# YannDubs/lossyless

Measured on AMD Instinct MI355X. Metric: encode_img_per_sec, higher is better.
Workload: dtype f16; 1 GPU; clip_compressor_b005 encode, synthetic 224x224x3 fp16 NHWC, batch=1024/GPU (configs[1]); batch_per_gpu=1024, layout=nhwc, vit_weights=synthetic-seed1, parallelism=image-parallel x1, entropy_group=16, tower_batch=8704, tower_streams=1, distinct_batches=9

## Files before the change

include/lossyless_amd.h:

```cpp
#ifndef LOSSYLESS_AMD_H
#define LOSSYLESS_AMD_H

#include <stddef.h>
#include <stdint.h>

#ifdef __cplusplus
extern "C" {
#endif

#define LLA_OK 0
#define LLA_EINVAL (-1)
#define LLA_ECAP (-2)
#define LLA_EHIP (-3)
#define LLA_EDATA (-4)

#define LLA_ABI_VERSION 4

int lla_abi_version(void);
const char *lla_source_sha(void);
int lla_last_hip_error(void);


int lla_pmf_to_quantized_cdf(const float *pmf, int n, int precision, uint32_t *cdf_out);

// ... 208 lines not shown
int lla_gemm_f32(const float *A, int lda, const float *W, int ldw, const float *bias, float *C, int ldc,
                 int M, int N, int K, int relu, void *stream);

size_t lla_svm_pass_workspace_bytes(int C, int K);
int lla_svm_pass(const void *z, int z_dtype, int ld_z, const int32_t *y, int B, int C, const float *W, const float *b,
                 const float *V, const float *vb, int K, int ld_w, float *out_W, float *out_b, double *out_loss,
                 int accumulate, void *workspace, void *stream);

size_t lla_svm_grid_pass_workspace_bytes(int C, int J);
int lla_svm_grid_pass(const void *z, int z_dtype, int ld_z, const int32_t *y, const int32_t *fold, int B, int C,
                      const float *W, const float *b, const float *V, const float *vb, int J, int ld_w,
                      const int32_t *col_class, const int32_t *col_held, const float *col_cpos, const float *col_cneg,
                      float *out_W, float *out_b, double *out_loss, int accumulate, void *workspace, void *stream);

size_t lla_softmax_pass_workspace_bytes(int C, int K, int B);
int lla_softmax_pass(const void *z, int z_dtype, int ld_z, const int32_t *y, int B, int C, const float *W, const float *b,
                     const float *V, const float *vb, int K, int ld_w, const float *class_weight, float *out_W,
                     float *out_b, double *out_loss, int accumulate, void *workspace, void *stream);

size_t lla_softmax_grid_pass_workspace_bytes(int C, int K, int G);
int lla_softmax_grid_pass(const void *z, int z_dtype, int ld_z, const int32_t *y, const int32_t *fold, int B, int C,
                          const float *W, const float *b, const float *V, const float *vb, int K, int G, int ld_w,
                          const int32_t *group_held, const float *group_class_weight, float *out_W, float *out_b,
                          double *out_loss, int accumulate, void *workspace, void *stream);


int lla_gemm_f32_nn(const float *dY, int ldy, const float *W, int ldw, const float *H, int ldh, float *dX, int ldx,
                    int M, int N, int K, void *stream);
int lla_gemm_f32_tn(const float *dY, int ldy, const float *X, int ldx, float *dW, int ldw, float *db, int M, int N, int K,
                    void *stream);
size_t lla_softmax_xent_workspace_bytes(int B);
int lla_softmax_xent(const float *logits, int ld, const int32_t *y, int B, int K, int Kpad, float scale, float *dlogits,
                     int ldd, double *out_loss, int32_t *out_correct, void *workspace, void *stream);
int lla_adamw_step(float *p, const float *g, float *m, float *v, long long n, double lr, double beta1, double beta2,
                   double eps, double weight_decay, double bias_correction1, double bias_correction2, void *stream);

int lla_conv3x3_relu_f16(const void *in, int n, int H, int W, int pitch, int cin, const void *weights,
                         const float *bias, void *out, int ldc, int cout, void *stream);
int lla_conv3x3_direct_relu_f16(const void *in, int n, int H, int W, int pitch, int cin, const void *weights, int kpad,
                                const void *bias, void *out, int ldc, int cout, int pool, void *stream);
int lla_rn50_bottleneck_f16(const void *x, int n, int H, int W, int pitch, int cin, const void *w1, int k1pad, const void *b1,
                            const void *w2, int k2pad, const void *b2, const void *w3, int k3pad, const void *b3, void *out,
                            int ldo, void *stream);
int lla_conv3x3_rgb_s2_relu_f16(const void *in, int n, int H, int W, const void *weights, int kpad, const void *bias,
                                void *out, int ldc, void *stream);
int lla_patch_embed_f16(const void *images, int layout, int B, const void *conv_w, const float *pos,
                        float *x, void *stream);
int lla_layernorm768(const float *x, size_t row_stride, const float *w, const float *b,
                     void *y16, int rows, void *stream);
size_t lla_gemm_resid_layernorm768_workspace_bytes(int M);
int lla_gemm_resid_layernorm768(const void *A, int lda, const void *W, const float *bias, float *x, const float *gamma,
                                const float *beta, void *h16, int M, int K, int wait_cycles, int rev, void *workspace,
                                void *stream);
int lla_attention50(const void *qkv, void *o, int B, void *stream);

size_t lla_rn50_weights_bytes(void);
int lla_rn50_conv_count(void);
int lla_rn50_conv_desc(int i, int64_t *out8);
int lla_rn50_fused_desc(int stage, int64_t *out8);
int lla_rn50_attnpool_offsets(int64_t *out7);
size_t lla_rn50_workspace_bytes(int chunk);
int lla_rn50_forward(const void *images_nhwc_f16, int B, const void *weights, void *workspace,
                     size_t workspace_bytes, int chunk, void *z_out, void *stream, void *tower);

#ifdef __cplusplus
}
#endif
#endif
```

lossyless_amd/_lib.py:

```python
import ctypes
import os

import torch

_HERE = os.path.dirname(os.path.abspath(__file__))
LIB_PATH = os.environ.get("LLA_LIB") or os.path.join(_HERE, "liblossyless_amd.so")

LLA_OK = 0
LLA_EINVAL, LLA_ECAP, LLA_EHIP, LLA_EDATA = -1, -2, -3, -4
ABI_VERSION = 4
LLA_Z_F16, LLA_Z_F32 = 1, 2
LLA_LAYOUT_NHWC, LLA_LAYOUT_NCHW = 0, 1
LLA_EPI_F16, LLA_EPI_QUICKGELU_F16, LLA_EPI_RESID_F32, LLA_EPI_RELU_F16, LLA_EPI_ADD_RELU_F16 = 0, 1, 2, 4, 5
_ERR = {-1: "LLA_EINVAL", -2: "LLA_ECAP", -3: "LLA_EHIP", -4: "LLA_EDATA"}

VIT_GLOBAL = dict(CONV1_NHWC=0, CONV1_NCHW=1, CLASS_EMB=2, POS_EMB=3, LN_PRE_W=4, LN_PRE_B=5,
                  LN_POST_W=6, LN_POST_B=7, PROJ_T=8)
VIT_LAYER = dict(LN1_W=16, LN1_B=17, QKV_W=18, QKV_B=19, OUT_W=20, OUT_B=21, LN2_W=22, LN2_B=23,
                 FC_W=24, FC_B=25, CPROJ_W=26, CPROJ_B=27)

_vp, _i, _sz = ctypes.c_void_p, ctypes.c_int, ctypes.c_size_t
_SIGNATURES = {
    "lla_abi_version": (_i, []),
    "lla_last_hip_error": (_i, []),
# ... 37 lines not shown
    "lla_preprocess_workspace_bytes": (_sz, [_i, _i]),
    "lla_preprocess_clip": (_i, [_vp, _i, _i, _i, _i, _i, _vp, _vp, _i, _vp, _vp, _i, _vp, _vp, _vp, _sz,
                                 _vp, _vp]),
    "lla_vit_b32_weights_bytes": (_sz, []),
    "lla_vit_b32_param_offset": (_sz, [_i, _i]),
    "lla_vit_b32_param_bytes": (_sz, [_i]),
    "lla_vit_b32_workspace_bytes": (_sz, [_i]),
    "lla_vit_b32_forward": (_i, [_vp, _i, _i, _vp, _vp, _sz, _i, _vp, _vp]),
    "lla_profiler_create": (_i, [ctypes.POINTER(ctypes.c_void_p), _i]),
    "lla_profiler_destroy": (_i, [_vp]),
    "lla_profiler_collect": (_i, [_vp, _vp, _vp, _vp]),
    "lla_vit_b32_forward_profiled": (_i, [_vp, _i, _i, _vp, _vp, _sz, _i, _vp, _vp, _vp]),
    "lla_tower_create": (_i, [ctypes.POINTER(ctypes.c_void_p)]),
    "lla_tower_destroy": (_i, [_vp]),
    "lla_tower_join": (_i, [_vp, _vp]),
    "lla_tower_set_option": (_i, [_vp, _i, _i]),
    "lla_vit_b32_forward_lanes": (_i, [_vp, _vp, _i, _i, _vp, _vp, _sz, _i, _vp, _vp, _i]),
    "lla_vit_b32_forward_gather": (_i, [_vp, _vp, _i, _i, _i, _i, _vp, _vp, _sz, _vp, _vp]),
    "lla_gemm_f16": (_i, [_vp, _vp, _vp, _vp, _i, _i, _i, _i, _vp]),
    "lla_patch_embed_f16": (_i, [_vp, _i, _i, _vp, _vp, _vp, _vp]),
    "lla_gemm_plan": (_i, [_i, _i, _i, _i, _i, _i, _i, _i, _i, _vp, _vp, _vp]),
    "lla_gemm_f16_ex": (_i, [_vp, _i, _vp, _vp, _vp, _i, _vp, _i, _i, _i, _i, _i, _vp]),
    "lla_gemm_f32": (_i, [_vp, _i, _vp, _i, _vp, _vp, _i, _i, _i, _i, _i, _vp]),
    "lla_svm_pass_workspace_bytes": (_sz, [_i, _i]),
    "lla_svm_pass": (_i, [_vp, _i, _i, _vp, _i, _i, _vp, _vp, _vp, _vp, _i, _i, _vp, _vp, _vp, _i, _vp, _vp]),
    "lla_svm_grid_pass_workspace_bytes": (_sz, [_i, _i]),
    "lla_svm_grid_pass": (_i, [_vp, _i, _i, _vp, _vp, _i, _i, _vp, _vp, _vp, _vp, _i, _i, _vp, _vp, _vp, _vp, _vp, _vp, _vp,
                               _i, _vp, _vp]),
    "lla_softmax_pass_workspace_bytes": (_sz, [_i, _i, _i]),
    "lla_softmax_pass": (_i, [_vp, _i, _i, _vp, _i, _i, _vp, _vp, _vp, _vp, _i, _i, _vp, _vp, _vp, _vp, _i, _vp, _vp]),
    "lla_softmax_grid_pass_workspace_bytes": (_sz, [_i, _i, _i]),
    "lla_softmax_grid_pass": (_i, [_vp, _i, _i, _vp, _vp, _i, _i, _vp, _vp, _vp, _vp, _i, _i, _i, _vp, _vp, _vp, _vp, _vp,
                                   _i, _vp, _vp]),
    "lla_gemm_f32_nn": (_i, [_vp, _i, _vp, _i, _vp, _i, _vp, _i, _i, _i, _i, _vp]),
    "lla_gemm_f32_tn": (_i, [_vp, _i, _vp, _i, _vp, _i, _vp, _i, _i, _i, _vp]),
    "lla_softmax_xent_workspace_bytes": (_sz, [_i]),
    "lla_softmax_xent": (_i, [_vp, _i, _vp, _i, _i, _i, ctypes.c_float, _vp, _i, _vp, _vp, _vp, _vp]),
    "lla_adamw_step": (_i, [_vp, _vp, _vp, _vp, ctypes.c_longlong] + [ctypes.c_double] * 7 + [_vp]),
    "lla_conv3x3_relu_f16": (_i, [_vp, _i, _i, _i, _i, _i, _vp, _vp, _vp, _i, _i, _vp]),
    "lla_conv3x3_direct_relu_f16": (_i, [_vp, _i, _i, _i, _i, _i, _vp, _i, _vp, _vp, _i, _i, _i, _vp]),
    "lla_conv3x3_rgb_s2_relu_f16": (_i, [_vp, _i, _i, _i, _vp, _i, _vp, _vp, _i, _vp]),
    "lla_rn50_bottleneck_f16": (_i, [_vp, _i, _i, _i, _i, _i, _vp, _i, _vp, _vp, _i, _vp, _vp, _i, _vp, _vp, _i, _vp]),
    "lla_rn50_weights_bytes": (_sz, []),
    "lla_rn50_conv_count": (_i, []),
    "lla_rn50_conv_desc": (_i, [_i, _vp]),
    "lla_rn50_fused_desc": (_i, [_i, _vp]),
    "lla_rn50_attnpool_offsets": (_i, [_vp]),
    "lla_rn50_workspace_bytes": (_sz, [_i]),
    "lla_rn50_forward": (_i, [_vp, _i, _vp, _vp, _sz, _i, _vp, _vp, _vp]),
    "lla_layernorm768": (_i, [_vp, _sz, _vp, _vp, _vp, _i, _vp]),
    "lla_gemm_resid_layernorm768_workspace_bytes": (_sz, [_i]),
    "lla_gemm_resid_layernorm768": (_i, [_vp, _i, _vp, _vp, _vp, _vp, _vp, _vp, _i, _i, _i, _i, _vp, _vp]),
    "lla_attention50": (_i, [_vp, _vp, _i, _vp]),
}
EXPORTS = tuple(sorted(_SIGNATURES))

_lib = None
_CSRC = os.path.join(_HERE, "csrc")


def tree_sha():
    script = os.path.join(_CSRC, "source_sha.py")
    if not os.path.exists(script):
        return None
    import importlib.util
    spec = importlib.util.spec_from_file_location("_lla_source_sha", script)
    mod = importlib.util.module_from_spec(spec)
    spec.loader.exec_module(mod)
    return mod.source_sha(_CSRC)


def built_sha(path=None):
    import re
    path = path or LIB_PATH
    if not os.path.exists(path):
        return None
    with open(path, "rb") as f:
        m = re.search(rb"LLA_SOURCE_SHA=([0-9a-f]{16})", f.read())
    return m.group(1).decode() if m else None


def stale(path=None):
    path = path or LIB_PATH
    if not os.path.exists(path):
        return f"{path} is missing"
    want, have = tree_sha(), built_sha(path)
    if want is not None and have != want:
        return f"{path} was built from sources {have}, the tree is {want}"
    return None


def ensure_built(path=None):
    import subprocess
    path = path or LIB_PATH
    why = stale(path)
    if why is None:
        return False
    name = os.path.basename(path)
    if os.path.dirname(os.path.abspath(path)) == os.path.join(_HERE, "variants"):
        raise RuntimeError(f"{why}: rebuild it with the DEFS it was made with (make -C lossyless_amd/csrc variant NAME=... DEFS=...)")
    target = {"liblossyless_amd.so": [], "liblossyless_amd_ablation.so": ["ablation"], "liblossyless_amd_probes.so": ["probes"]}.get(name)
    if target is None or _lib is not None:
        raise RuntimeError(why)
    subprocess.check_call(["make", "-j8", "-C", _CSRC, *target])
    return True

# ... 83 lines not shown
```

lossyless_amd/csrc/layernorm_attention.hip:

```cpp
#include "tower_kernels.h"

namespace lla {
namespace {

__device__ __forceinline__ float wave_sum(float v) { return wave_sum_f32(v); }

struct Row768 {
  float4 v[3];
};

#ifndef LLA_LN_LOAD
#define LLA_LN_LOAD 0
#endif
__device__ __forceinline__ Row768 load_row768(const float *row, int lane) {
  Row768 in;
  const float4 *src = reinterpret_cast<const float4 *>(row) + lane;
#if LLA_LN_LOAD == 0
#pragma unroll
  for (int i = 0; i < 3; ++i) in.v[i] = src[64 * i];
#elif LLA_LN_LOAD == 1
  asm volatile("global_load_dwordx4 %0, %3, off sc1\n\t"
               "global_load_dwordx4 %1, %3, off offset:1024 sc1\n\t"
               "global_load_dwordx4 %2, %3, off offset:2048 sc1\n\t"
               "s_waitcnt vmcnt(0)"
// ... 18 lines not shown
  float t[3], u[3];
#pragma unroll
  for (int i = 0; i < 3; ++i) {
    t[i] = wave_sum((x.v[i].x + x.v[i].y) + (x.v[i].z + x.v[i].w));
    u[i] = wave_sum((x.v[i].x * x.v[i].x + x.v[i].y * x.v[i].y) + (x.v[i].z * x.v[i].z + x.v[i].w * x.v[i].w));
  }
  ln_finish((t[0] + t[1]) + t[2], (u[0] + u[1]) + u[2], mean, rstd);
}

__device__ __forceinline__ Row768 row_affine(const Row768 &x, float mean, float rstd,
                                             const float *__restrict__ w,
                                             const float *__restrict__ b, int lane) {
  Row768 y;
#pragma unroll
  for (int i = 0; i < 3; ++i) {
    const float4 g = reinterpret_cast<const float4 *>(w)[lane + 64 * i];
    const float4 o = reinterpret_cast<const float4 *>(b)[lane + 64 * i];
    y.v[i].x = ln_affine(x.v[i].x, mean, rstd, g.x, o.x);
    y.v[i].y = ln_affine(x.v[i].y, mean, rstd, g.y, o.y);
    y.v[i].z = ln_affine(x.v[i].z, mean, rstd, g.z, o.z);
    y.v[i].w = ln_affine(x.v[i].w, mean, rstd, g.w, o.w);
  }
  return y;
}

__device__ __forceinline__ void store_row_f16(f16 *dst, const Row768 &y, int lane) {
#pragma unroll
  for (int i = 0; i < 3; ++i) {
    f16x4 h;
    h[0] = (f16)y.v[i].x; h[1] = (f16)y.v[i].y; h[2] = (f16)y.v[i].z; h[3] = (f16)y.v[i].w;
    reinterpret_cast<f16x4 *>(dst)[lane + 64 * i] = h;
  }
}

__global__ __launch_bounds__(256) void layernorm768_kernel(const float *__restrict__ x,
                                                           size_t row_stride,
                                                           const float *__restrict__ w,
                                                           const float *__restrict__ b,
                                                           f16 *__restrict__ y, int rows, int rev) {
  kernel_acquire();
  const int blk = rev ? gridDim.x - 1 - blockIdx.x : blockIdx.x;
  const int row = blk * 4 + (threadIdx.x >> 6);
  const int lane = threadIdx.x & 63;
  if (row >= rows) return;
  const Row768 in = load_row768(x + (size_t)row * row_stride, lane);
  float mean, rstd;
  row_stats(in, mean, rstd);
  const Row768 out = row_affine(in, mean, rstd, w, b, lane);
  store_row_f16(y + (size_t)row * kWidth, out, lane);
  kernel_release();
}

#ifndef LLA_LNX_CLEANUP_SPLIT
#define LLA_LNX_CLEANUP_SPLIT 8
#endif
static_assert(64 % LLA_LNX_CLEANUP_SPLIT == 0 && (64 / LLA_LNX_CLEANUP_SPLIT) % 4 == 0,
              "lnx_cleanup_kernel: a wave takes 64 / split rows, four at a time");
__global__ __launch_bounds__(256) void lnx_cleanup_kernel(const float *__restrict__ x, const unsigned *__restrict__ done,
                                                          const float *__restrict__ w, const float *__restrict__ b,
                                                          f16 *__restrict__ y, int rev, unsigned epoch, int split) {
  kernel_acquire();
#if LLA_LNX_FENCE & 2
  __builtin_amdgcn_fence(__ATOMIC_ACQUIRE, "agent");
#endif
  const int blk = rev ? gridDim.x - 1 - blockIdx.x : blockIdx.x;
  const int rt = blk / split;
  const bool complete = __hip_atomic_load(done + rt * 3, __ATOMIC_RELAXED, __HIP_MEMORY_SCOPE_AGENT) == epoch &&
                        __hip_atomic_load(done + rt * 3 + 1, __ATOMIC_RELAXED, __HIP_MEMORY_SCOPE_AGENT) == epoch &&
                        __hip_atomic_load(done + rt * 3 + 2, __ATOMIC_RELAXED, __HIP_MEMORY_SCOPE_AGENT) == epoch;
  if (complete) return;
  const int lane = threadIdx.x & 63;
  const int per_wave = 64 / split;
  const int row0 = rt * 256 + (blk - rt * split) * (256 / split) + (threadIdx.x >> 6) * per_wave;
  for (int r0 = 0; r0 < per_wave; r0 += 4) {
    f32x4 raw[4][3];
#pragma unroll
    for (int r = 0; r < 4; ++r) {
      const float4 *src = reinterpret_cast<const float4 *>(x + (size_t)(row0 + r0 + r) * kWidth) + lane;
      asm volatile("global_load_dwordx4 %0, %3, off\n\t"
                   "global_load_dwordx4 %1, %3, off offset:1024\n\t"
                   "global_load_dwordx4 %2, %3, off offset:2048"
                   : "=&v"(raw[r][0]), "=&v"(raw[r][1]), "=&v"(raw[r][2]) : "v"(src) : "memory");
    }
    asm volatile("s_waitcnt vmcnt(0)" : "+v"(raw[0][0]), "+v"(raw[0][1]), "+v"(raw[0][2]), "+v"(raw[1][0]), "+v"(raw[1][1]),
                 "+v"(raw[1][2]), "+v"(raw[2][0]), "+v"(raw[2][1]), "+v"(raw[2][2]), "+v"(raw[3][0]), "+v"(raw[3][1]),
                 "+v"(raw[3][2])::"memory");
#pragma unroll
    for (int r = 0; r < 4; ++r) {
      Row768 in;
#pragma unroll
      for (int i = 0; i < 3; ++i) in.v[i] = make_float4(raw[r][i][0], raw[r][i][1], raw[r][i][2], raw[r][i][3]);
      float mean, rstd;
      row_stats(in, mean, rstd);
      store_row_f16(y + (size_t)(row0 + r0 + r) * kWidth, row_affine(in, mean, rstd, w, b, lane), lane);
    }
  }
  kernel_release();
}

__global__ __launch_bounds__(256) void ln_pre_ln1_kernel(
    float *__restrict__ x, const float *__restrict__ cls, const float *__restrict__ pos,
    const float *__restrict__ wpre, const float *__restrict__ bpre, const float *__restrict__ w1,
    const float *__restrict__ b1, f16 *__restrict__ h, int rows) {
  kernel_acquire();
  const int row = blockIdx.x * 4 + (threadIdx.x >> 6);
  const int lane = threadIdx.x & 63;
  if (row >= rows) return;
  float4 *xr = reinterpret_cast<float4 *>(x + (size_t)row * kWidth);
  Row768 in;
  if (row % kTokens == 0) {
#pragma unroll
    for (int i = 0; i < 3; ++i) {
      const float4 c = reinterpret_cast<const float4 *>(cls)[lane + 64 * i];
      const float4 q = reinterpret_cast<const float4 *>(pos)[lane + 64 * i];
      in.v[i] = make_float4(c.x + q.x, c.y + q.y, c.z + q.z, c.w + q.w);
    }
  } else {
    in = load_row768(x + (size_t)row * kWidth, lane);
  }
  float mean, rstd;
  row_stats(in, mean, rstd);
  const Row768 t = row_affine(in, mean, rstd, wpre, bpre, lane);
#pragma unroll
  for (int i = 0; i < 3; ++i) xr[lane + 64 * i] = t.v[i];
  row_stats(t, mean, rstd);
  const Row768 u = row_affine(t, mean, rstd, w1, b1, lane);
  store_row_f16(h + (size_t)row * kWidth, u, lane);
  kernel_release();
}


constexpr int kVPitch = 72;
#ifndef LLA_ATTN_LOAD
#define LLA_ATTN_LOAD 0
#endif
#if LLA_ATTN_LOAD == 2
#define LLA_ATTN_SC " sc1"
#elif LLA_ATTN_LOAD == 3
#define LLA_ATTN_SC " sc0 sc1"
#else
#define LLA_ATTN_SC ""
#endif

__global__ __launch_bounds__(256, 4) void attention50_kernel(const f16 *__restrict__ qkv,
                                                          f16 *__restrict__ o, int B, int rev) {
  kernel_acquire();
  __shared__ __attribute__((aligned(16))) f16 lds[4][64 * kVPitch];
  const int wid = threadIdx.x >> 6, lane = threadIdx.x & 63;
  const int r32 = lane & 31, hk = lane >> 5;
  const int blk = rev ? gridDim.x - 1 - blockIdx.x : blockIdx.x;
  const int b = blk / 3;
  const int head = (blk - b * 3) * 4 + wid;
  f16 *vs = lds[wid];
  const f16 *base = qkv + (size_t)b * kTokens * (3 * kWidth) + head * kHeadDim;
  const f16x8 zero8 = {0, 0, 0, 0, 0, 0, 0, 0};

  f16x8 kf[2][4], qf[2][4];
#if LLA_ATTN_LOAD
  {
    f16x8 vv[8];
#pragma unroll
    for (int it = 0; it < 8; ++it) {
      const int id = lane + 64 * it, j = id >> 3, dc = id & 7;
      const f16 *src = base + (size_t)(j < kTokens ? j : 0) * (3 * kWidth) + 2 * kWidth + dc * 8;
      asm volatile("global_load_dwordx4 %0, %1, off" LLA_ATTN_SC : "=v"(vv[it]) : "v"(src) : "memory");
    }
#pragma unroll
    for (int t = 0; t < 2; ++t) {
      const int row = 32 * t + r32;
      const f16 *rp = base + (size_t)(row < kTokens ? row : 0) * (3 * kWidth) + 8 * hk;
#pragma unroll
      for (int s = 0; s < 4; ++s) {
        asm volatile("global_load_dwordx4 %0, %1, off" LLA_ATTN_SC : "=v"(qf[t][s]) : "v"(rp + 16 * s) : "memory");
        asm volatile("global_load_dwordx4 %0, %1, off" LLA_ATTN_SC : "=v"(kf[t][s]) : "v"(rp + kWidth + 16 * s) : "memory");
      }
    }
    asm volatile("s_waitcnt vmcnt(0)"
                 : "+v"(vv[0]), "+v"(vv[1]), "+v"(vv[2]), "+v"(vv[3]), "+v"(vv[4]), "+v"(vv[5]), "+v"(vv[6]), "+v"(vv[7]),
                   "+v"(qf[0][0]), "+v"(qf[0][1]), "+v"(qf[0][2]), "+v"(qf[0][3]), "+v"(qf[1][0]), "+v"(qf[1][1]),
                   "+v"(qf[1][2]), "+v"(qf[1][3]), "+v"(kf[0][0]), "+v"(kf[0][1]), "+v"(kf[0][2]), "+v"(kf[0][3]),
                   "+v"(kf[1][0]), "+v"(kf[1][1]), "+v"(kf[1][2]), "+v"(kf[1][3])
                 :: "memory");
#pragma unroll
    for (int it = 0; it < 8; ++it) {
      const int id = lane + 64 * it, j = id >> 3, dc = id & 7;
      *reinterpret_cast<f16x8 *>(vs + j * kVPitch + dc * 8) = j < kTokens ? vv[it] : zero8;
    }
#pragma unroll
    for (int s = 0; s < 4; ++s)
      if (32 + r32 >= kTokens) { qf[1][s] = zero8; kf[1][s] = zero8; }
  }
#else
#pragma unroll
  for (int it = 0; it < 8; ++it) {
    const int id = lane + 64 * it, j = id >> 3, dc = id & 7;
    f16x8 v = zero8;
    if (j < kTokens)
      v = *reinterpret_cast<const f16x8 *>(base + (size_t)j * (3 * kWidth) + 2 * kWidth + dc * 8);
    *reinterpret_cast<f16x8 *>(vs + j * kVPitch + dc * 8) = v;
  }

#pragma unroll
  for (int t = 0; t < 2; ++t) {
    const int row = 32 * t + r32;
    const bool ok = row < kTokens;
    const f16 *rp = base + (size_t)(ok ? row : 0) * (3 * kWidth) + 8 * hk;
#pragma unroll
    for (int s = 0; s < 4; ++s) {
      qf[t][s] = ok ? *reinterpret_cast<const f16x8 *>(rp + 16 * s) : zero8;
      kf[t][s] = ok ? *reinterpret_cast<const f16x8 *>(rp + kWidth + 16 * s) : zero8;
    }
  }
#endif

  f32x16 sT[2][2];
#pragma unroll
  for (int jt = 0; jt < 2; ++jt)
#pragma unroll
    for (int it = 0; it < 2; ++it) {
#pragma unroll
      for (int r = 0; r < 16; ++r) sT[jt][it][r] = 0.f;
#pragma unroll
      for (int s = 0; s < 4; ++s)
        sT[jt][it] = __builtin_amdgcn_mfma_f32_32x32x16_f16(kf[jt][s], qf[it][s], sT[jt][it], 0, 0, 0);
    }

  f16x8 pf[2][2][2];
#pragma unroll
  for (int it = 0; it < 2; ++it) {
    float mx = -3.0e38f;
#pragma unroll
    for (int jt = 0; jt < 2; ++jt)
#pragma unroll
      for (int r = 0; r < 16; ++r) {
        const int j = 32 * jt + (r & 3) + 8 * (r >> 2) + 4 * hk;
        const float s = j < kTokens ? sT[jt][it][r] * 0.125f : -3.0e38f;
        sT[jt][it][r] = s;
        mx = fmaxf(mx, s);
      }
    {
      float lo, hi;
      half_wave_pair_f32(mx, lo, hi);
      mx = fmaxf(lo, hi);
    }
    float sum = 0.f;
#pragma unroll
    for (int jt = 0; jt < 2; ++jt)
#pragma unroll
      for (int r = 0; r < 16; ++r) {
        const int j = 32 * jt + (r & 3) + 8 * (r >> 2) + 4 * hk;
        const float e = j < kTokens ? __expf(sT[jt][it][r] - mx) : 0.f;
        sT[jt][it][r] = e;
        sum += e;
      }
    {
      float lo, hi;
      half_wave_pair_f32(sum, lo, hi);
      sum = lo + hi;
    }
    const float inv = 1.f / sum;
#pragma unroll
    for (int jt = 0; jt < 2; ++jt)
#pragma unroll
      for (int sp = 0; sp < 2; ++sp)
#pragma unroll
        for (int e = 0; e < 8; ++e) pf[it][jt][sp][e] = (f16)(sT[jt][it][8 * sp + e] * inv);
  }

  __syncthreads();

  f32x16 oT[2][2];
#pragma unroll
  for (int dt = 0; dt < 2; ++dt)
#pragma unroll
    for (int it = 0; it < 2; ++it)
#pragma unroll
      for (int r = 0; r < 16; ++r) oT[dt][it][r] = 0.f;
#pragma unroll
  for (int jt = 0; jt < 2; ++jt)
#pragma unroll
    for (int sp = 0; sp < 2; ++sp) {
#pragma unroll
      for (int dt = 0; dt < 2; ++dt) {
        f16x8 vf;
#pragma unroll
        for (int e = 0; e < 8; ++e) {
          const int j = 32 * jt + 16 * sp + (e & 3) + 8 * (e >> 2) + 4 * hk;
          vf[e] = vs[j * kVPitch + 32 * dt + r32];
        }
#pragma unroll
        for (int it = 0; it < 2; ++it)
          oT[dt][it] = __builtin_amdgcn_mfma_f32_32x32x16_f16(vf, pf[it][jt][sp], oT[dt][it], 0, 0, 0);
      }
    }

  __syncthreads();
#pragma unroll
  for (int dt = 0; dt < 2; ++dt)
#pragma unroll
    for (int it = 0; it < 2; ++it)
#pragma unroll
      for (int g = 0; g < 4; ++g) {
        f16x4 q4;
#pragma unroll
        for (int e = 0; e < 4; ++e) q4[e] = (f16)oT[dt][it][4 * g + e];
        *reinterpret_cast<f16x4 *>(vs + (32 * it + r32) * kVPitch + 32 * dt + 8 * g + 4 * hk) = q4;
      }
  __syncthreads();
  f16 *ob = o + (size_t)b * kTokens * kWidth + head * kHeadDim;
#pragma unroll
  for (int it = 0; it < 7; ++it) {
    const int id = lane + 64 * it, i = id >> 3, dc = id & 7;
    if (i < kTokens)
      *reinterpret_cast<f16x8 *>(ob + (size_t)i * kWidth + dc * 8) =
          *reinterpret_cast<const f16x8 *>(vs + i * kVPitch + dc * 8);
  }
  kernel_release();
}

}

int layernorm_impl(const float *x, size_t row_stride, const float *w, const float *b, void *y16, int rows, hipStream_t st,
                   Profiler *prof, int rev) {
  if (rows < 0 || row_stride < (size_t)kWidth || (row_stride & 3u)) return LLA_EINVAL;
  if (rows == 0) return LLA_OK;
  if (!x || !w || !b || !y16) return LLA_EINVAL;
  ProfScope scope(prof, st, LLA_PROF_LAYERNORM, (double)rows * kWidth * 6.0);
  layernorm768_kernel<<<(rows + 3) / 4, 256, 0, st>>>(x, row_stride, w, b, reinterpret_cast<f16 *>(y16), rows, rev);
  return check_launch();
}

int attention_impl(const void *qkv, void *o, int B, hipStream_t st, Profiler *prof, int rev) {
  if (B < 0) return LLA_EINVAL;
  if (B == 0) return LLA_OK;
  if (!qkv || !o) return LLA_EINVAL;
  ProfScope scope(prof, st, LLA_PROF_ATTENTION, (double)B * 12 * 4.0 * kTokens * kTokens * kHeadDim);
  attention50_kernel<<<B * 3, 256, 0, st>>>(reinterpret_cast<const f16 *>(qkv), reinterpret_cast<f16 *>(o), B, rev);
  return check_launch();
}

int ln_pre_ln1_impl(float *x, const float *cls, const float *pos, const float *wpre, const float *bpre, const float *w1,
                    const float *b1, void *h16, int rows, hipStream_t st, Profiler *prof) {
  ProfScope scope(prof, st, LLA_PROF_LAYERNORM, (double)rows * kWidth * 10.0);
  ln_pre_ln1_kernel<<<(rows + 3) / 4, 256, 0, st>>>(x, cls, pos, wpre, bpre, w1, b1, reinterpret_cast<f16 *>(h16), rows);
  return check_launch();
}

int lnx_cleanup_impl(const float *x, const unsigned *done, const float *w, const float *b, void *y16, int tiles_m, int rev,
                     unsigned epoch, hipStream_t st, Profiler *prof) {
  ProfScope scope(prof, st, LLA_PROF_LAYERNORM, 0.0);
  const int split = LLA_LNX_CLEANUP_SPLIT;
  lnx_cleanup_kernel<<<tiles_m * split, 256, 0, st>>>(x, done, w, b, reinterpret_cast<f16 *>(y16), rev, epoch, split);
  return check_launch();
}

}

using namespace lla;

extern "C" {

int lla_layernorm768(const float *x, size_t row_stride, const float *w, const float *b, void *y16, int rows, void *stream) {
  return layernorm_impl(x, row_stride, w, b, y16, rows, as_stream(stream), nullptr);
}

int lla_attention50(const void *qkv, void *o, int B, void *stream) {
  return attention_impl(qkv, o, B, as_stream(stream), nullptr);
}

}
```

lossyless_amd/csrc/tower.hip:

```cpp
#include "gemm_launch.h"
#include "switches.h"
#include "tower_kernels.h"

#include <atomic>
#include <cstdlib>
#include <map>
#include <mutex>

namespace lla {
namespace {

constexpr size_t kAlign = 256;
constexpr size_t align_up(size_t v) { return (v + kAlign - 1) & ~(kAlign - 1); }

size_t param_bytes(int id) {
  switch (id) {
    case LLA_VIT_CONV1_NHWC:
    case LLA_VIT_CONV1_NCHW: return (size_t)kWidth * kPatchK * 2;
    case LLA_VIT_CLASS_EMB: return kWidth * 4;
    case LLA_VIT_POS_EMB: return (size_t)kTokens * kWidth * 4;
    case LLA_VIT_LN_PRE_W: case LLA_VIT_LN_PRE_B:
    case LLA_VIT_LN_POST_W: case LLA_VIT_LN_POST_B: return kWidth * 4;
    case LLA_VIT_PROJ_T: return (size_t)kOut * kWidth * 2;
    case LLA_VIT_LN1_W: case LLA_VIT_LN1_B: case LLA_VIT_LN2_W: case LLA_VIT_LN2_B:
// ... 272 lines not shown
static unsigned next_lnx_epoch() {
  static std::atomic<unsigned> counter{0x5EED0000u};
  unsigned e = counter.fetch_add(1u, std::memory_order_relaxed) + 1u;
  return e ? e : counter.fetch_add(1u, std::memory_order_relaxed) + 1u;
}

static int resid_layernorm_gemm(GemmParams g, const float *gamma, const float *beta, f16 *h, float *part, unsigned *words,
                                int wait, int cleanup_rev, hipStream_t st, Profiler *prof) {
  const int tiles_m = g.M / 256;
  g.lnx_g = gamma; g.lnx_b = beta; g.lnx_h = h; g.lnx_part = part;
  g.lnx_flag = words;
  g.lnx_done = words + (size_t)tiles_m * 3;
  g.lnx_wait = wait;
  g.lnx_epoch = next_lnx_epoch();
  {
    ProfScope scope(prof, st, LLA_PROF_GEMM, 2.0 * g.M * g.N * g.K);
    const int rc2 = launch_q4(EPI_RESID_LNX, g, st);
    if (rc2 != LLA_OK) return rc2;
  }
#if LLA_LNX_SYNC
  if (hipStreamSynchronize(st) != hipSuccess) return hip_fail(hipGetLastError());
#endif
  return lnx_cleanup_impl(reinterpret_cast<const float *>(g.C), g.lnx_done, gamma, beta, h, tiles_m, cleanup_rev, g.lnx_epoch,
                          st, prof);
}

size_t lla_gemm_resid_layernorm768_workspace_bytes(int M) {
  if (M <= 0 || (M & 255)) return 0;
  return (size_t)(M / 256) * (3 * 256 * 16 + 6 * sizeof(unsigned));
}

int lla_gemm_resid_layernorm768(const void *A, int lda, const void *W, const float *bias, float *x, const float *gamma,
                                const float *beta, void *h16, int M, int K, int wait_cycles, int rev, void *workspace,
                                void *stream) {
  GemmParams g{};
  g.A = reinterpret_cast<const f16 *>(A);
  g.W = reinterpret_cast<const f16 *>(W);
  g.bias = bias;
  g.C = x;
  g.M = M; g.N = kWidth; g.K = K; g.lda = lda; g.ldc = kWidth;
  g.rev = rev;
  if (!q4_takes(gemm_shape(EPI_RESID_LNX, A_PLAIN, g)) || (rev != 0 && rev != 1)) return LLA_EINVAL;
  if (!A || !W || !x || !gamma || !beta || !h16 || !workspace) return LLA_EINVAL;
  auto misaligned = [](const void *p) { return (reinterpret_cast<uintptr_t>(p) & 15u) != 0; };
  if (misaligned(A) || misaligned(W) || misaligned(bias) || misaligned(x) || misaligned(gamma) || misaligned(beta) ||
      misaligned(h16) || misaligned(workspace))
    return LLA_EINVAL;
  const int tiles_m = M / 256;
  float *const part = reinterpret_cast<float *>(workspace);
  unsigned *const words = reinterpret_cast<unsigned *>(part + (size_t)tiles_m * 3 * 256 * 4);
  hipStream_t st = as_stream(stream);
  if (hipMemsetAsync(words, 0, (size_t)tiles_m * 6 * sizeof(unsigned), st) != hipSuccess) return hip_fail(hipGetLastError());
  return resid_layernorm_gemm(g, gamma, beta, reinterpret_cast<f16 *>(h16), part, words, wait_cycles, rev ^ 1, st, nullptr);
}

int lla_tower_set_option(void *tower, int option, int value) {
  Lanes *l = reinterpret_cast<Lanes *>(tower);
  if (!l) return LLA_EINVAL;
  switch (option) {
    case LLA_TOWER_OPT_LNX: l->lnx = value != 0; return LLA_OK;
    case LLA_TOWER_OPT_LNX_WAIT: l->lnx_wait = value; return LLA_OK;
    default: return LLA_EINVAL;
  }
}

int lla_tower_join(void *tower, void *stream) {
  if (!tower) return LLA_EINVAL;
  return lanes_join(reinterpret_cast<Lanes *>(tower), as_stream(stream));
}

int lla_vit_b32_forward(const void *images, int layout, int B, const void *weights,
                        void *workspace, size_t ws_bytes, int chunk, void *z_out, void *stream) {
  return vit_forward_impl(images, layout, B, weights, workspace, ws_bytes, chunk, z_out, stream, nullptr, nullptr,
                          false);
}

int lla_vit_b32_forward_profiled(const void *images, int layout, int B, const void *weights,
                                 void *workspace, size_t ws_bytes, int chunk, void *z_out,
                                 void *stream, void *profiler) {
  return vit_forward_impl(images, layout, B, weights, workspace, ws_bytes, chunk, z_out, stream, profiler, nullptr,
                          false);
}

int lla_vit_b32_forward_lanes(void *tower, const void *images, int layout, int B, const void *weights,
                              void *workspace, size_t ws_bytes, int chunk, void *z_out, void *stream,
                              int deferred) {
  if (!tower) return LLA_EINVAL;
  return vit_forward_impl(images, layout, B, weights, workspace, ws_bytes, chunk, z_out, stream, nullptr,
                          reinterpret_cast<Lanes *>(tower), deferred != 0);
}

int lla_vit_b32_forward_gather(void *tower, const void *const *pieces, int n_pieces, int piece_images, int layout, int B,
                               const void *weights, void *workspace, size_t ws_bytes, void *z_out, void *stream) {
  if (!tower || !pieces) return LLA_EINVAL;
  return vit_forward_impl(nullptr, layout, B, weights, workspace, ws_bytes, 0, z_out, stream, nullptr,
                          reinterpret_cast<Lanes *>(tower), false, pieces, n_pieces, piece_images);
}

static int vit_forward_impl(const void *images, int layout, int B, const void *weights, void *workspace,
                            size_t ws_bytes, int chunk, void *z_out, void *stream, void *profiler,
                            Lanes *tower, bool deferred, const void *const *pieces, int n_pieces, int piece_images) {
  Profiler *prof = reinterpret_cast<Profiler *>(profiler);
  if (pieces) {
    if (n_pieces < 1 || n_pieces > 64 || piece_images <= 0 || (piece_images & 255) || B <= (n_pieces - 1) * piece_images ||
        B > n_pieces * piece_images || (B & 127) || B < 256)
      return LLA_EINVAL;
// ... 76 lines not shown
    pe.C = ws.x;
    pe.pos = P32(LLA_VIT_POS_EMB, 0);
    pe.M = bc * kPatches; pe.N = kWidth; pe.K = kPatchK; pe.lda = 0; pe.ldc = kWidth;
    if (pieces) {
      if (lanes != 1 || c0 != 0 || bc != B) return LLA_EINVAL;
      pe.a_chunk_images = piece_images;
      for (int i = 0; i < n_pieces; ++i) pe.a_chunk[i] = reinterpret_cast<const f16 *>(pieces[i]);
    }
    LLA_TRY(launch_gemm_rt(EPI_PATCH, layout == LLA_LAYOUT_NHWC ? A_PATCH_NHWC : A_PATCH_NCHW, pe, st, prof));
    LLA_TRY(ln_pre_ln1_impl(ws.x, P32(LLA_VIT_CLASS_EMB, 0), P32(LLA_VIT_POS_EMB, 0), P32(LLA_VIT_LN_PRE_W, 0),
                            P32(LLA_VIT_LN_PRE_B, 0), P32(LLA_VIT_LN1_W, 0), P32(LLA_VIT_LN1_B, 0), ws.h, M, st, prof));

    int dir = 0;
    const int zig = sw::zigzag();
    const bool lnx = M >= kBigM && q4_takes({EPI_RESID_LNX, A_PLAIN, M, kWidth, kMlp, kMlp, kWidth, 0, 0}) && (!tower || tower->lnx);
    const int tiles_m = M / 256;
    float *const lnx_part = ws.part;
    unsigned *const lnx_words = reinterpret_cast<unsigned *>(ws.part + (size_t)tiles_m * 3 * 256 * 4);
    int lnx_launch = 0;
    if (lnx && hipMemsetAsync(lnx_words, 0, (size_t)(2 * kLayers - 1) * tiles_m * 6 * sizeof(unsigned), st) != hipSuccess)
      return hip_fail(hipGetLastError());
    auto lnx_gemm = [&](GemmParams g, const float *gamma, const float *beta, int &d) -> int {
      unsigned *const words = lnx_words + (size_t)lnx_launch * tiles_m * 6;
      ++lnx_launch;
      d ^= zig; g.rev = d;
      d ^= zig;
      return resid_layernorm_gemm(g, gamma, beta, ws.xh, lnx_part, words, tower ? tower->lnx_wait : kLnxWaitDefault, d, st, prof);
    };
    bool ln1_by_gemm = false;
    for (int l = 0; l < kLayers; ++l) {
      if (l > 0 && !ln1_by_gemm) {
        dir ^= zig;
        LLA_TRY(layernorm_impl(ws.x, kWidth, P32(LLA_VIT_LN1_W, l), P32(LLA_VIT_LN1_B, l), ws.h, M, st, prof, dir));
      }
      GemmParams g{};
      g.M = M;
      const bool cls_only = (l == kLayers - 1) && sw::prune_last_block();
      g.A = ln1_by_gemm ? ws.xh : ws.h; g.W = P16(LLA_VIT_QKV_W, l); g.bias = P32(LLA_VIT_QKV_B, l); g.C = ws.big;
      g.N = 3 * kWidth; g.K = kWidth; g.lda = kWidth; g.ldc = 3 * kWidth;
      if (cls_only) {
        GemmParams kv = g;
        kv.W = g.W + (size_t)kWidth * kWidth; kv.bias = g.bias + kWidth;
        kv.C = ws.big + kWidth; kv.N = 2 * kWidth;
        GemmParams q = g;
        q.M = bc; q.N = kWidth; q.lda = kTokens * kWidth; q.ldc = kTokens * 3 * kWidth;
        LLA_TRY(launch_gemm_rt(EPI_F16, A_PLAIN, kv, st, prof));
        LLA_TRY(launch_gemm_rt(EPI_F16, A_PLAIN, q, st, prof));
      } else {
        dir ^= zig; g.rev = dir;
        LLA_TRY(launch_gemm_rt(EPI_F16, A_PLAIN, g, st, prof));
        g.rev = 0;
      }
      dir ^= zig;
      LLA_TRY(attention_impl(ws.big, ws.h, bc, st, prof, dir));
      const int rows = cls_only ? bc : M;
      const int xs = cls_only ? kTokens * kWidth : kWidth;
      g.M = rows;
      g.A = ws.h; g.W = P16(LLA_VIT_OUT_W, l); g.bias = P32(LLA_VIT_OUT_B, l); g.C = ws.x;
      g.N = kWidth; g.K = kWidth; g.lda = xs; g.ldc = xs;
      const bool ln2_by_gemm = lnx && !cls_only;
      if (ln2_by_gemm) {
        LLA_TRY(lnx_gemm(g, P32(LLA_VIT_LN2_W, l), P32(LLA_VIT_LN2_B, l), dir));
      } else {
        dir ^= zig; g.rev = dir;
        LLA_TRY(launch_gemm_rt(EPI_RESID, A_PLAIN, g, st, prof));
        g.rev = 0;
        dir ^= zig;
        LLA_TRY(layernorm_impl(ws.x, (size_t)xs, P32(LLA_VIT_LN2_W, l), P32(LLA_VIT_LN2_B, l), ws.h, rows, st, prof, dir));
      }
      g.A = ln2_by_gemm ? ws.xh : ws.h; g.W = P16(LLA_VIT_FC_W, l); g.bias = P32(LLA_VIT_FC_B, l); g.C = ws.big;
      g.N = kMlp; g.K = kWidth; g.lda = kWidth; g.ldc = kMlp;
      dir ^= zig; g.rev = dir;
      LLA_TRY(launch_gemm_rt(EPI_QGELU, A_PLAIN, g, st, prof));
      g.rev = 0;
      g.A = ws.big; g.W = P16(LLA_VIT_CPROJ_W, l); g.bias = P32(LLA_VIT_CPROJ_B, l); g.C = ws.x;
      g.N = kWidth; g.K = kMlp; g.lda = kMlp; g.ldc = xs;
      ln1_by_gemm = lnx && !cls_only && l + 1 < kLayers;
      if (ln1_by_gemm) {
        LLA_TRY(lnx_gemm(g, P32(LLA_VIT_LN1_W, l + 1), P32(LLA_VIT_LN1_B, l + 1), dir));
      } else {
        dir ^= zig; g.rev = dir;
        LLA_TRY(launch_gemm_rt(EPI_RESID, A_PLAIN, g, st, prof));
        g.rev = 0;
      }
    }

    LLA_TRY(layernorm_impl(ws.x, (size_t)kTokens * kWidth, P32(LLA_VIT_LN_POST_W, 0),
                           P32(LLA_VIT_LN_POST_B, 0), ws.h, bc, st, prof));
    GemmParams g{};
    g.A = ws.h; g.W = P16(LLA_VIT_PROJ_T, 0); g.bias = nullptr;
    g.C = reinterpret_cast<f16 *>(z_out) + (size_t)c0 * kOut;
    g.M = bc; g.N = kOut; g.K = kWidth; g.lda = kWidth; g.ldc = kOut;
    LLA_TRY(launch_gemm_rt(EPI_F16, A_PLAIN, g, st, prof));
  }
#undef LLA_TRY
  if (lanes == 2 && deferred) { ln->next = slice & 1; ln->dirty = true; return LLA_OK; }
  if (lanes == 2) return lanes_join(ln, st_caller);
  return LLA_OK;
}

}
```

lossyless_amd/csrc/tower_kernels.h:

```cpp
#pragma once
#include "gemm_common.h"

namespace lla {

int layernorm_impl(const float *x, size_t row_stride, const float *w, const float *b, void *y16, int rows, hipStream_t st,
                   Profiler *prof, int rev = 0);
int attention_impl(const void *qkv, void *o, int B, hipStream_t st, Profiler *prof, int rev = 0);
int ln_pre_ln1_impl(float *x, const float *cls, const float *pos, const float *wpre, const float *bpre, const float *w1,
                    const float *b1, void *h16, int rows, hipStream_t st, Profiler *prof);
int lnx_cleanup_impl(const float *x, const unsigned *done, const float *w, const float *b, void *y16, int tiles_m, int rev,
                     unsigned epoch, hipStream_t st, Profiler *prof);

}
```

Measured before the change: 108,300 img/s.

## Compact LN cleanup work list and add class-token-only attention for last layer

The LN cleanup kernel now runs a fixed-size persistent grid. It scans the per-tile done flags, builds a compacted list of incomplete tiles in shared memory, and shares the remaining row chunks out across blocks, instead of launching one block per tile chunk that mostly exits early. Attention also gains a class-only template variant for the pruned last block, which computes only the class-token query row and writes just that output. This cuts launch overhead and wasted attention work, but the new scan loop adds extra syncs per block.

```diff
diff --git a/include/lossyless_amd.h b/include/lossyless_amd.h
--- a/include/lossyless_amd.h
+++ b/include/lossyless_amd.h
@@ -284,7 +284,10 @@
 int lla_gemm_resid_layernorm768(const void *A, int lda, const void *W, const float *bias, float *x, const float *gamma,
                                 const float *beta, void *h16, int M, int K, int wait_cycles, int rev, void *workspace,
                                 void *stream);
+int lla_lnx_cleanup(const float *x, const unsigned *done, const float *gamma, const float *beta, void *h16, int tiles_m,
+                    int rev, unsigned epoch, void *stream);
 int lla_attention50(const void *qkv, void *o, int B, void *stream);
+int lla_attention50_class(const void *qkv, void *o, int B, void *stream);
 
 size_t lla_rn50_weights_bytes(void);
 int lla_rn50_conv_count(void);
diff --git a/lossyless_amd/_lib.py b/lossyless_amd/_lib.py
--- a/lossyless_amd/_lib.py
+++ b/lossyless_amd/_lib.py
@@ -113,6 +113,8 @@
     "lla_gemm_resid_layernorm768_workspace_bytes": (_sz, [_i]),
     "lla_gemm_resid_layernorm768": (_i, [_vp, _i, _vp, _vp, _vp, _vp, _vp, _vp, _i, _i, _i, _i, _vp, _vp]),
     "lla_attention50": (_i, [_vp, _vp, _i, _vp]),
+    "lla_attention50_class": (_i, [_vp, _vp, _i, _vp]),
+    "lla_lnx_cleanup": (_i, [_vp, _vp, _vp, _vp, _vp, _i, _i, ctypes.c_uint, _vp]),
 }
 EXPORTS = tuple(sorted(_SIGNATURES))
 
diff --git a/lossyless_amd/csrc/layernorm_attention.hip b/lossyless_amd/csrc/layernorm_attention.hip
--- a/lossyless_amd/csrc/layernorm_attention.hip
+++ b/lossyless_amd/csrc/layernorm_attention.hip
@@ -94,48 +94,89 @@
 }
 
 #ifndef LLA_LNX_CLEANUP_SPLIT
-#define LLA_LNX_CLEANUP_SPLIT 8
+#define LLA_LNX_CLEANUP_SPLIT 16
+#endif
+#ifndef LLA_LNX_CLEANUP_GRID
+#define LLA_LNX_CLEANUP_GRID 256
 #endif
 static_assert(64 % LLA_LNX_CLEANUP_SPLIT == 0 && (64 / LLA_LNX_CLEANUP_SPLIT) % 4 == 0,
               "lnx_cleanup_kernel: a wave takes 64 / split rows, four at a time");
+constexpr int kLnxScan = 2048;
 __global__ __launch_bounds__(256) void lnx_cleanup_kernel(const float *__restrict__ x, const unsigned *__restrict__ done,
                                                           const float *__restrict__ w, const float *__restrict__ b,
-                                                          f16 *__restrict__ y, int rev, unsigned epoch, int split) {
+                                                          f16 *__restrict__ y, int tiles_m, int rev, unsigned epoch) {
   kernel_acquire();
 #if LLA_LNX_FENCE & 2
   __builtin_amdgcn_fence(__ATOMIC_ACQUIRE, "agent");
 #endif
-  const int blk = rev ? gridDim.x - 1 - blockIdx.x : blockIdx.x;
-  const int rt = blk / split;
-  const bool complete = __hip_atomic_load(done + rt * 3, __ATOMIC_RELAXED, __HIP_MEMORY_SCOPE_AGENT) == epoch &&
-                        __hip_atomic_load(done + rt * 3 + 1, __ATOMIC_RELAXED, __HIP_MEMORY_SCOPE_AGENT) == epoch &&
-                        __hip_atomic_load(done + rt * 3 + 2, __ATOMIC_RELAXED, __HIP_MEMORY_SCOPE_AGENT) == epoch;
-  if (complete) return;
-  const int lane = threadIdx.x & 63;
-  const int per_wave = 64 / split;
-  const int row0 = rt * 256 + (blk - rt * split) * (256 / split) + (threadIdx.x >> 6) * per_wave;
-  for (int r0 = 0; r0 < per_wave; r0 += 4) {
-    f32x4 raw[4][3];
-#pragma unroll
-    for (int r = 0; r < 4; ++r) {
-      const float4 *src = reinterpret_cast<const float4 *>(x + (size_t)(row0 + r0 + r) * kWidth) + lane;
-      asm volatile("global_load_dwordx4 %0, %3, off\n\t"
-                   "global_load_dwordx4 %1, %3, off offset:1024\n\t"
-                   "global_load_dwordx4 %2, %3, off offset:2048"
-                   : "=&v"(raw[r][0]), "=&v"(raw[r][1]), "=&v"(raw[r][2]) : "v"(src) : "memory");
-    }
-    asm volatile("s_waitcnt vmcnt(0)" : "+v"(raw[0][0]), "+v"(raw[0][1]), "+v"(raw[0][2]), "+v"(raw[1][0]), "+v"(raw[1][1]),
-                 "+v"(raw[1][2]), "+v"(raw[2][0]), "+v"(raw[2][1]), "+v"(raw[2][2]), "+v"(raw[3][0]), "+v"(raw[3][1]),
-                 "+v"(raw[3][2])::"memory");
-#pragma unroll
-    for (int r = 0; r < 4; ++r) {
-      Row768 in;
-#pragma unroll
-      for (int i = 0; i < 3; ++i) in.v[i] = make_float4(raw[r][i][0], raw[r][i][1], raw[r][i][2], raw[r][i][3]);
-      float mean, rstd;
-      row_stats(in, mean, rstd);
-      store_row_f16(y + (size_t)(row0 + r0 + r) * kWidth, row_affine(in, mean, rstd, w, b, lane), lane);
-    }
+  __shared__ unsigned short list[kLnxScan];
+  __shared__ int wave_count[kLnxScan / 64];
+  constexpr int split = LLA_LNX_CLEANUP_SPLIT, per_wave = 64 / split;
+  const int tid = threadIdx.x, wid = tid >> 6, lane = tid & 63;
+  int seen = 0;
+  for (int u0 = 0; u0 < tiles_m; u0 += kLnxScan) {
+    unsigned d[kLnxScan / 256][3];
+#pragma unroll
+    for (int r = 0; r < kLnxScan / 256; ++r) {
+      const int u = u0 + r * 256 + tid;
+      const int rt = u < tiles_m ? (rev ? tiles_m - 1 - u : u) : 0;
+#pragma unroll
+      for (int k = 0; k < 3; ++k) d[r][k] = __hip_atomic_load(done + rt * 3 + k, __ATOMIC_RELAXED, __HIP_MEMORY_SCOPE_AGENT);
+    }
+    unsigned long long todo[kLnxScan / 256];
+#pragma unroll
+    for (int r = 0; r < kLnxScan / 256; ++r) {
+      const bool complete = d[r][0] == epoch && d[r][1] == epoch && d[r][2] == epoch;
+      todo[r] = __ballot(u0 + r * 256 + tid < tiles_m && !complete);
+      if (lane == 0) wave_count[r * 4 + wid] = __popcll(todo[r]);
+    }
+    __syncthreads();
+    int n = 0;
+#pragma unroll
+    for (int r = 0; r < kLnxScan / 256; ++r) {
+      int before = 0;
+#pragma unroll
+      for (int wv = 0; wv < 4; ++wv) {
+        if (wv == wid) before = n;
+        n += wave_count[r * 4 + wv];
+      }
+      if ((todo[r] >> lane) & 1ull)
+        list[before + __popcll(todo[r] & ((1ull << lane) - 1ull))] = (unsigned short)(r * 256 + tid);
+    }
+    __syncthreads();
+    const int grid = gridDim.x;
+    int first = ((int)blockIdx.x - (int)(((long long)seen * split) % grid)) % grid;
+    if (first < 0) first += grid;
+    for (int item = first; item < n * split; item += grid) {
+      const int u = u0 + list[item / split], part = item % split;
+      const int rt = rev ? tiles_m - 1 - u : u;
+      const int row0 = rt * 256 + (rev ? split - 1 - part : part) * (256 / split) + wid * per_wave;
+      for (int r0 = 0; r0 < per_wave; r0 += 4) {
+        f32x4 raw[4][3];
+#pragma unroll
+        for (int r = 0; r < 4; ++r) {
+          const float4 *src = reinterpret_cast<const float4 *>(x + (size_t)(row0 + r0 + r) * kWidth) + lane;
+          asm volatile("global_load_dwordx4 %0, %3, off\n\t"
+                       "global_load_dwordx4 %1, %3, off offset:1024\n\t"
+                       "global_load_dwordx4 %2, %3, off offset:2048"
+                       : "=&v"(raw[r][0]), "=&v"(raw[r][1]), "=&v"(raw[r][2]) : "v"(src) : "memory");
+        }
+        asm volatile("s_waitcnt vmcnt(0)" : "+v"(raw[0][0]), "+v"(raw[0][1]), "+v"(raw[0][2]), "+v"(raw[1][0]), "+v"(raw[1][1]),
+                     "+v"(raw[1][2]), "+v"(raw[2][0]), "+v"(raw[2][1]), "+v"(raw[2][2]), "+v"(raw[3][0]), "+v"(raw[3][1]),
+                     "+v"(raw[3][2])::"memory");
+#pragma unroll
+        for (int r = 0; r < 4; ++r) {
+          Row768 in;
+#pragma unroll
+          for (int i = 0; i < 3; ++i) in.v[i] = make_float4(raw[r][i][0], raw[r][i][1], raw[r][i][2], raw[r][i][3]);
+          float mean, rstd;
+          row_stats(in, mean, rstd);
+          store_row_f16(y + (size_t)(row0 + r0 + r) * kWidth, row_affine(in, mean, rstd, w, b, lane), lane);
+        }
+      }
+    }
+    seen += n;
+    __syncthreads();
   }
   kernel_release();
 }
@@ -184,10 +225,13 @@
 #define LLA_ATTN_SC ""
 #endif
 
+template <bool kClassOnly>
 __global__ __launch_bounds__(256, 4) void attention50_kernel(const f16 *__restrict__ qkv,
                                                           f16 *__restrict__ o, int B, int rev) {
   kernel_acquire();
-  __shared__ __attribute__((aligned(16))) f16 lds[4][64 * kVPitch];
+  constexpr int kQT = kClassOnly ? 1 : 2;
+  constexpr int kVRows = kClassOnly ? kTokens : 64;
+  __shared__ __attribute__((aligned(16))) f16 lds[4][kVRows * kVPitch];
   const int wid = threadIdx.x >> 6, lane = threadIdx.x & 63;
   const int r32 = lane & 31, hk = lane >> 5;
   const int blk = rev ? gridDim.x - 1 - blockIdx.x : blockIdx.x;
@@ -213,7 +257,12 @@
       const f16 *rp = base + (size_t)(row < kTokens ? row : 0) * (3 * kWidth) + 8 * hk;
 #pragma unroll
       for (int s = 0; s < 4; ++s) {
-        asm volatile("global_load_dwordx4 %0, %1, off" LLA_ATTN_SC : "=v"(qf[t][s]) : "v"(rp + 16 * s) : "memory");
+        if (t < kQT) {
+          const f16 *qp = kClassOnly ? base + 8 * hk : rp;
+          asm volatile("global_load_dwordx4 %0, %1, off" LLA_ATTN_SC : "=v"(qf[t][s]) : "v"(qp + 16 * s) : "memory");
+        } else {
+          qf[t][s] = zero8;
+        }
         asm volatile("global_load_dwordx4 %0, %1, off" LLA_ATTN_SC : "=v"(kf[t][s]) : "v"(rp + kWidth + 16 * s) : "memory");
       }
     }
@@ -226,11 +275,13 @@
 #pragma unroll
     for (int it = 0; it < 8; ++it) {
       const int id = lane + 64 * it, j = id >> 3, dc = id & 7;
-      *reinterpret_cast<f16x8 *>(vs + j * kVPitch + dc * 8) = j < kTokens ? vv[it] : zero8;
-    }
-#pragma unroll
-    for (int s = 0; s < 4; ++s)
+      if (j < kVRows) *reinterpret_cast<f16x8 *>(vs + j * kVPitch + dc * 8) = j < kTokens ? vv[it] : zero8;
+    }
+#pragma unroll
+    for (int s = 0; s < 4; ++s) {
       if (32 + r32 >= kTokens) { qf[1][s] = zero8; kf[1][s] = zero8; }
+      if (kClassOnly && r32 != 0) qf[0][s] = zero8;
+    }
   }
 #else
 #pragma unroll
@@ -239,7 +290,7 @@
     f16x8 v = zero8;
     if (j < kTokens)
       v = *reinterpret_cast<const f16x8 *>(base + (size_t)j * (3 * kWidth) + 2 * kWidth + dc * 8);
-    *reinterpret_cast<f16x8 *>(vs + j * kVPitch + dc * 8) = v;
+    if (j < kVRows) *reinterpret_cast<f16x8 *>(vs + j * kVPitch + dc * 8) = v;
   }
 
 #pragma unroll
@@ -249,7 +300,10 @@
     const f16 *rp = base + (size_t)(ok ? row : 0) * (3 * kWidth) + 8 * hk;
 #pragma unroll
     for (int s = 0; s < 4; ++s) {
-      qf[t][s] = ok ? *reinterpret_cast<const f16x8 *>(rp + 16 * s) : zero8;
+      if (kClassOnly)
+        qf[t][s] = (t == 0 && r32 == 0) ? *reinterpret_cast<const f16x8 *>(rp + 16 * s) : zero8;
+      else
+        qf[t][s] = ok ? *reinterpret_cast<const f16x8 *>(rp + 16 * s) : zero8;
       kf[t][s] = ok ? *reinterpret_cast<const f16x8 *>(rp + kWidth + 16 * s) : zero8;
     }
   }
@@ -259,7 +313,7 @@
 #pragma unroll
   for (int jt = 0; jt < 2; ++jt)
 #pragma unroll
-    for (int it = 0; it < 2; ++it) {
+    for (int it = 0; it < kQT; ++it) {
 #pragma unroll
       for (int r = 0; r < 16; ++r) sT[jt][it][r] = 0.f;
 #pragma unroll
@@ -269,7 +323,7 @@
 
   f16x8 pf[2][2][2];
 #pragma unroll
-  for (int it = 0; it < 2; ++it) {
+  for (int it = 0; it < kQT; ++it) {
     float mx = -3.0e38f;
 #pragma unroll
     for (int jt = 0; jt < 2; ++jt)
@@ -315,7 +369,7 @@
 #pragma unroll
   for (int dt = 0; dt < 2; ++dt)
 #pragma unroll
-    for (int it = 0; it < 2; ++it)
+    for (int it = 0; it < kQT; ++it)
 #pragma unroll
       for (int r = 0; r < 16; ++r) oT[dt][it][r] = 0.f;
 #pragma unroll
@@ -328,10 +382,13 @@
 #pragma unroll
         for (int e = 0; e < 8; ++e) {
           const int j = 32 * jt + 16 * sp + (e & 3) + 8 * (e >> 2) + 4 * hk;
-          vf[e] = vs[j * kVPitch + 32 * dt + r32];
+          if (kClassOnly)
+            vf[e] = j < kTokens ? vs[j * kVPitch + 32 * dt + r32] : (f16)0;
+          else
+            vf[e] = vs[j * kVPitch + 32 * dt + r32];
         }
 #pragma unroll
-        for (int it = 0; it < 2; ++it)
+        for (int it = 0; it < kQT; ++it)
           oT[dt][it] = __builtin_amdgcn_mfma_f32_32x32x16_f16(vf, pf[it][jt][sp], oT[dt][it], 0, 0, 0);
       }
     }
@@ -340,22 +397,27 @@
 #pragma unroll
   for (int dt = 0; dt < 2; ++dt)
 #pragma unroll
-    for (int it = 0; it < 2; ++it)
+    for (int it = 0; it < kQT; ++it)
 #pragma unroll
       for (int g = 0; g < 4; ++g) {
         f16x4 q4;
 #pragma unroll
         for (int e = 0; e < 4; ++e) q4[e] = (f16)oT[dt][it][4 * g + e];
-        *reinterpret_cast<f16x4 *>(vs + (32 * it + r32) * kVPitch + 32 * dt + 8 * g + 4 * hk) = q4;
+        if (!kClassOnly || r32 == 0)
+          *reinterpret_cast<f16x4 *>(vs + (32 * it + r32) * kVPitch + 32 * dt + 8 * g + 4 * hk) = q4;
       }
   __syncthreads();
   f16 *ob = o + (size_t)b * kTokens * kWidth + head * kHeadDim;
-#pragma unroll
-  for (int it = 0; it < 7; ++it) {
-    const int id = lane + 64 * it, i = id >> 3, dc = id & 7;
-    if (i < kTokens)
-      *reinterpret_cast<f16x8 *>(ob + (size_t)i * kWidth + dc * 8) =
-          *reinterpret_cast<const f16x8 *>(vs + i * kVPitch + dc * 8);
+  if (kClassOnly) {
+    if (lane < 8) *reinterpret_cast<f16x8 *>(ob + lane * 8) = *reinterpret_cast<const f16x8 *>(vs + lane * 8);
+  } else {
+#pragma unroll
+    for (int it = 0; it < 7; ++it) {
+      const int id = lane + 64 * it, i = id >> 3, dc = id & 7;
+      if (i < kTokens)
+        *reinterpret_cast<f16x8 *>(ob + (size_t)i * kWidth + dc * 8) =
+            *reinterpret_cast<const f16x8 *>(vs + i * kVPitch + dc * 8);
+    }
   }
   kernel_release();
 }
@@ -372,12 +434,15 @@
   return check_launch();
 }
 
-int attention_impl(const void *qkv, void *o, int B, hipStream_t st, Profiler *prof, int rev) {
+int attention_impl(const void *qkv, void *o, int B, hipStream_t st, Profiler *prof, int rev, bool class_only) {
   if (B < 0) return LLA_EINVAL;
   if (B == 0) return LLA_OK;
   if (!qkv || !o) return LLA_EINVAL;
-  ProfScope scope(prof, st, LLA_PROF_ATTENTION, (double)B * 12 * 4.0 * kTokens * kTokens * kHeadDim);
-  attention50_kernel<<<B * 3, 256, 0, st>>>(reinterpret_cast<const f16 *>(qkv), reinterpret_cast<f16 *>(o), B, rev);
+  ProfScope scope(prof, st, LLA_PROF_ATTENTION, (double)B * 12 * 4.0 * (class_only ? 1 : kTokens) * kTokens * kHeadDim);
+  if (class_only)
+    attention50_kernel<true><<<B * 3, 256, 0, st>>>(reinterpret_cast<const f16 *>(qkv), reinterpret_cast<f16 *>(o), B, rev);
+  else
+    attention50_kernel<false><<<B * 3, 256, 0, st>>>(reinterpret_cast<const f16 *>(qkv), reinterpret_cast<f16 *>(o), B, rev);
   return check_launch();
 }
 
@@ -391,8 +456,9 @@
 int lnx_cleanup_impl(const float *x, const unsigned *done, const float *w, const float *b, void *y16, int tiles_m, int rev,
                      unsigned epoch, hipStream_t st, Profiler *prof) {
   ProfScope scope(prof, st, LLA_PROF_LAYERNORM, 0.0);
-  const int split = LLA_LNX_CLEANUP_SPLIT;
-  lnx_cleanup_kernel<<<tiles_m * split, 256, 0, st>>>(x, done, w, b, reinterpret_cast<f16 *>(y16), rev, epoch, split);
+  const long long items = (long long)tiles_m * LLA_LNX_CLEANUP_SPLIT;
+  const int grid = items < LLA_LNX_CLEANUP_GRID ? (int)items : LLA_LNX_CLEANUP_GRID;
+  lnx_cleanup_kernel<<<grid, 256, 0, st>>>(x, done, w, b, reinterpret_cast<f16 *>(y16), tiles_m, rev, epoch);
   return check_launch();
 }
 
@@ -410,4 +476,8 @@
   return attention_impl(qkv, o, B, as_stream(stream), nullptr);
 }
 
-}
+int lla_attention50_class(const void *qkv, void *o, int B, void *stream) {
+  return attention_impl(qkv, o, B, as_stream(stream), nullptr, 0, true);
+}
+
+}
diff --git a/lossyless_amd/csrc/tower.hip b/lossyless_amd/csrc/tower.hip
--- a/lossyless_amd/csrc/tower.hip
+++ b/lossyless_amd/csrc/tower.hip
@@ -348,6 +348,16 @@
   hipStream_t st = as_stream(stream);
   if (hipMemsetAsync(words, 0, (size_t)tiles_m * 6 * sizeof(unsigned), st) != hipSuccess) return hip_fail(hipGetLastError());
   return resid_layernorm_gemm(g, gamma, beta, reinterpret_cast<f16 *>(h16), part, words, wait_cycles, rev ^ 1, st, nullptr);
+}
+
+int lla_lnx_cleanup(const float *x, const unsigned *done, const float *gamma, const float *beta, void *h16, int tiles_m,
+                    int rev, unsigned epoch, void *stream) {
+  if (tiles_m <= 0 || (long long)tiles_m * 256 * kWidth >= (1ll << 32) || (rev != 0 && rev != 1)) return LLA_EINVAL;
+  if (!x || !done || !gamma || !beta || !h16) return LLA_EINVAL;
+  auto misaligned = [](const void *p) { return (reinterpret_cast<uintptr_t>(p) & 15u) != 0; };
+  if (misaligned(x) || misaligned(gamma) || misaligned(beta) || misaligned(h16) || (reinterpret_cast<uintptr_t>(done) & 3u))
+    return LLA_EINVAL;
+  return lnx_cleanup_impl(x, done, gamma, beta, h16, tiles_m, rev, epoch, as_stream(stream), nullptr);
 }
 
 int lla_tower_set_option(void *tower, int option, int value) {
@@ -530,7 +540,7 @@
         g.rev = 0;
       }
       dir ^= zig;
-      LLA_TRY(attention_impl(ws.big, ws.h, bc, st, prof, dir));
+      LLA_TRY(attention_impl(ws.big, ws.h, bc, st, prof, dir, cls_only));
       const int rows = cls_only ? bc : M;
       const int xs = cls_only ? kTokens * kWidth : kWidth;
       g.M = rows;
diff --git a/lossyless_amd/csrc/tower_kernels.h b/lossyless_amd/csrc/tower_kernels.h
--- a/lossyless_amd/csrc/tower_kernels.h
+++ b/lossyless_amd/csrc/tower_kernels.h
@@ -5,7 +5,7 @@
 
 int layernorm_impl(const float *x, size_t row_stride, const float *w, const float *b, void *y16, int rows, hipStream_t st,
                    Profiler *prof, int rev = 0);
-int attention_impl(const void *qkv, void *o, int B, hipStream_t st, Profiler *prof, int rev = 0);
+int attention_impl(const void *qkv, void *o, int B, hipStream_t st, Profiler *prof, int rev = 0, bool class_only = false);
 int ln_pre_ln1_impl(float *x, const float *cls, const float *pos, const float *wpre, const float *bpre, const float *w1,
                     const float *b1, void *h16, int rows, hipStream_t st, Profiler *prof);
 int lnx_cleanup_impl(const float *x, const unsigned *done, const float *w, const float *b, void *y16, int tiles_m, int rev,
```

After: 108,700 img/s (median of 6 runs). No clear change (+0.4%).
